# daxiongpro/EPNet

Hardware: AMD Instinct MI355X
Metric: SA-stack points/sec per GPU (16384-pt KITTI scene) + % HBM roofline (higher is better)
Workload: dtype f32

## Files before the change

### epnet_amd/csrc/group.hip

```cpp

#include <type_traits>

#include "common.h"
#include "spatial.h"
#include "runsum.h"

namespace epnet {

constexpr int kGThreads = 256;
constexpr int kGChan = 16;

__global__ __launch_bounds__(kGThreads) void gather_rows_vec4_kernel(int c, int n, int p, size_t ostride,
                                                                     const float *__restrict__ points,
                                                                     const int *__restrict__ idx,
                                                                     float *__restrict__ out) {
    int wg_x, wg_y, bs;
    xcd_scene_map3(wg_x, wg_y, bs);
    const int c0 = wg_y * kGChan;
    const int q4 = wg_x * kGThreads + threadIdx.x;
    if (q4 * 4 >= p) return;
    const int4 id = *reinterpret_cast<const int4 *>(idx + (size_t)bs * p + (size_t)q4 * 4);
    const int cend = min(c, c0 + kGChan);
    const float *src = points + ((size_t)bs * c + c0) * n;
    float *dst = out + (size_t)bs * ostride + (size_t)c0 * p + (size_t)q4 * 4;
// ... 224 lines not shown
#pragma unroll 1
        for (int set = 0; set < 2; ++set) {
            const int p = set ? p1 : p0;
            const int *ix = (set ? idx1 : idx0) + (size_t)bs * p;
            float *dst_base = (set ? out1 : out0) + (size_t)bs * (set ? ostride1 : ostride0) + (size_t)c0 * p;
            if (p > 0) serve_span<QUAD, decltype(g)::value, decltype(u)::value>(s_rows, nr, n, ix, 0, p, dst_base, p);
        }
    });
}

__global__ __launch_bounds__(kGThreads) void scatter_rows_lds_kernel(int c, int n, int p, int rows, size_t gstride,
                                                                     const float *__restrict__ grad_out,
                                                                     const int *__restrict__ idx,
                                                                     float *__restrict__ grad_points) {
    extern __shared__ float acc[];
    const int bs = blockIdx.y;
    const int c0 = blockIdx.x * rows;
    const int nr = min(rows, c - c0);
    for (int e = threadIdx.x; e < nr * n; e += kGThreads) acc[e] = 0.f;
    __syncthreads();
    const int *ix = idx + (size_t)bs * p;
    const float *go = grad_out + (size_t)bs * gstride + (size_t)c0 * p;
    for (int q = threadIdx.x; q < p; q += kGThreads) {
        const int id = ix[q];
        for (int r = 0; r < nr; ++r) atomicAdd(&acc[r * n + id], go[(size_t)r * p + q]);
    }
    __syncthreads();
    float *gp = grad_points + ((size_t)bs * c + c0) * n;
    for (int e = threadIdx.x; e < nr * n; e += kGThreads) gp[e] += acc[e];
}

__global__ __launch_bounds__(kGThreads) void scatter_rows_atomic_kernel(int c, int n, int p, size_t gstride,
                                                                        const float *__restrict__ grad_out,
                                                                        const int *__restrict__ idx,
                                                                        float *__restrict__ grad_points) {
    const int bs = blockIdx.z, ci = blockIdx.y;
    const int q = blockIdx.x * kGThreads + threadIdx.x;
    if (q >= p) return;
    atomicAdd(grad_points + ((size_t)bs * c + ci) * n + idx[(size_t)bs * p + q],
              grad_out[(size_t)bs * gstride + (size_t)ci * p + q]);
}

__global__ __launch_bounds__(kGThreads) void group_xyz_centred_kernel(int n, int npoints, int nsample, size_t ostride,
                                                                      const float *__restrict__ xyz,
                                                                      const float *__restrict__ new_xyz,
                                                                      const int *__restrict__ idx, float *__restrict__ out) {
    int wg_x, bs;
    xcd_scene_map(wg_x, bs);
    const int p = npoints * nsample;
    const int q = wg_x * kGThreads + threadIdx.x;
    if (q >= p) return;
    const int id = idx[(size_t)bs * p + q];
    const int ci = q / nsample;
    const float *pt = xyz + ((size_t)bs * n + id) * 3;
    const float *ce = new_xyz + ((size_t)bs * npoints + ci) * 3;
    float *dst = out + (size_t)bs * ostride + q;
    dst[0] = pt[0] - ce[0];
    dst[(size_t)p] = pt[1] - ce[1];
    dst[(size_t)p * 2] = pt[2] - ce[2];
}

__global__ __launch_bounds__(kGThreads) void group_xyz_centred_vec4_kernel(int n, int npoints, int nsample, size_t ostride,
                                                                           const float *__restrict__ xyz,
                                                                           const float *__restrict__ new_xyz,
                                                                           const int *__restrict__ idx,
                                                                           float *__restrict__ out) {
    int wg_x, bs;
    xcd_scene_map(wg_x, bs);
    const int p = npoints * nsample;
    const int q = (wg_x * kGThreads + threadIdx.x) * 4;
    if (q >= p) return;
    const int4 id = *reinterpret_cast<const int4 *>(idx + (size_t)bs * p + q);
    const float *base = xyz + (size_t)bs * n * 3;
    const float *ce = new_xyz + ((size_t)bs * npoints + q / nsample) * 3;
    const float cx = ce[0], cy = ce[1], cz = ce[2];
    const float *p0 = base + (size_t)id.x * 3, *p1 = base + (size_t)id.y * 3, *p2 = base + (size_t)id.z * 3,
                *p3 = base + (size_t)id.w * 3;
    float *dst = out + (size_t)bs * ostride + q;
    *reinterpret_cast<float4 *>(dst) = make_float4(p0[0] - cx, p1[0] - cx, p2[0] - cx, p3[0] - cx);
    *reinterpret_cast<float4 *>(dst + (size_t)p) = make_float4(p0[1] - cy, p1[1] - cy, p2[1] - cy, p3[1] - cy);
    *reinterpret_cast<float4 *>(dst + (size_t)p * 2) = make_float4(p0[2] - cz, p1[2] - cz, p2[2] - cz, p3[2] - cz);
}

__global__ __launch_bounds__(kGLdsThreads) void group_linear_lds_kernel(int c, int n, int npoints, int nsample, int rows, int tile,
                                                                        const float *__restrict__ z, const float *__restrict__ xyz,
                                                                        const float *__restrict__ new_xyz, const int *__restrict__ idx,
                                                                        const float *__restrict__ wx, const float *__restrict__ bias,
                                                                        float *__restrict__ out) {
    extern __shared__ float s_rows[];
    const int bs = blockIdx.z;
    const int c0 = blockIdx.y * rows;
    const int nr = min(rows, c - c0);
    const int p = npoints * nsample;
    const float *src = z + ((size_t)bs * c + c0) * n;
    const int total = nr * n;
    if ((n & 3) == 0 && ((uintptr_t)src & 15) == 0) {
        const float4 *src4 = reinterpret_cast<const float4 *>(src);
        float4 *dst4 = reinterpret_cast<float4 *>(s_rows);
        EPNET_STAGE_PRAGMA
        for (int e = threadIdx.x; e < total / 4; e += kGLdsThreads) dst4[e] = src4[e];
    } else {
        for (int e = threadIdx.x; e < total; e += kGLdsThreads) s_rows[e] = src[e];
    }
    __syncthreads();
    const int q_begin = blockIdx.x * tile, q_end = min(p, q_begin + tile);
    const int *ix = idx + (size_t)bs * p;
    const float *pts = xyz + (size_t)bs * n * 3;
    float *dst_base = out + ((size_t)bs * c + c0) * p;
    for (int q = q_begin + threadIdx.x * 4; q < q_end; q += kGLdsThreads * 4) {
        const int4 id = *reinterpret_cast<const int4 *>(ix + q);
        const float *ce = new_xyz + ((size_t)bs * npoints + q / nsample) * 3;
        const float cx = ce[0], cy = ce[1], cz = ce[2];
        const float *p0 = pts + (size_t)id.x * 3, *p1 = pts + (size_t)id.y * 3, *p2 = pts + (size_t)id.z * 3, *p3 = pts + (size_t)id.w * 3;
        const float dx0 = p0[0] - cx, dy0 = p0[1] - cy, dz0 = p0[2] - cz;
        const float dx1 = p1[0] - cx, dy1 = p1[1] - cy, dz1 = p1[2] - cz;
        const float dx2 = p2[0] - cx, dy2 = p2[1] - cy, dz2 = p2[2] - cz;
        const float dx3 = p3[0] - cx, dy3 = p3[1] - cy, dz3 = p3[2] - cz;
        float *dst = dst_base + q;
        const float *row = s_rows;
#pragma unroll 2
        for (int r = 0; r < nr; ++r) {
            const float w0 = wx[(c0 + r) * 3], w1 = wx[(c0 + r) * 3 + 1], w2 = wx[(c0 + r) * 3 + 2];
            float4 v;
            v.x = row[id.x] + (w0 * dx0 + w1 * dy0 + w2 * dz0);
            v.y = row[id.y] + (w0 * dx1 + w1 * dy1 + w2 * dz1);
            v.z = row[id.z] + (w0 * dx2 + w1 * dy2 + w2 * dz2);
            v.w = row[id.w] + (w0 * dx3 + w1 * dy3 + w2 * dz3);
            if (bias) {
                const float bv = bias[c0 + r];
                v.x += bv; v.y += bv; v.z += bv; v.w += bv;
            }
            store_stream(dst, v.x, v.y, v.z, v.w);
            row += n;
            dst += p;
        }
    }
}

__global__ __launch_bounds__(kGThreads) void group_linear_scalar_kernel(int c, int n, int npoints, int nsample,
                                                                        const float *__restrict__ z, const float *__restrict__ xyz,
                                                                        const float *__restrict__ new_xyz, const int *__restrict__ idx,
                                                                        const float *__restrict__ wx, const float *__restrict__ bias,
                                                                        float *__restrict__ out) {
    const int bs = blockIdx.z;
    const int c0 = blockIdx.y * kGChan;
    const int p = npoints * nsample;
    const int q = blockIdx.x * kGThreads + threadIdx.x;
    if (q >= p) return;
    const int id = idx[(size_t)bs * p + q];
    const float *pt = xyz + ((size_t)bs * n + id) * 3;
    const float *ce = new_xyz + ((size_t)bs * npoints + q / nsample) * 3;
    const float dx = pt[0] - ce[0], dy = pt[1] - ce[1], dz = pt[2] - ce[2];
    const int cend = min(c, c0 + kGChan);
    for (int ci = c0; ci < cend; ++ci) {
        float v = z[((size_t)bs * c + ci) * n + id] + (wx[ci * 3] * dx + wx[ci * 3 + 1] * dy + wx[ci * 3 + 2] * dz);
        if (bias) v += bias[ci];
        out[((size_t)bs * c + ci) * p + q] = v;
    }
}

constexpr int kGwRows = 8;
__global__ __launch_bounds__(kGThreads) void group_linear_grad_w_kernel(int c, int n, int npoints, int nsample, int tile,
                                                                        const float *__restrict__ grad_out,
                                                                        const float *__restrict__ xyz,
                                                                        const float *__restrict__ new_xyz,
                                                                        const int *__restrict__ idx, float *__restrict__ grad_w) {
// ... 258 lines not shown
}

static int launch_group_xyz(int b, int n, int npoints, int nsample, long long p, size_t ostride, const float *xyz,
                            const float *new_xyz, const int *idx, float *out, hipStream_t s) {
    if (nsample % 4 == 0 && (((uintptr_t)idx | (uintptr_t)out) % 16 == 0) && (ostride % 4 == 0))
        hipLaunchKernelGGL(group_xyz_centred_vec4_kernel, dim3((unsigned)div_up64(p / 4, kGThreads), b), dim3(kGThreads), 0, s, n,
                           npoints, nsample, ostride, xyz, new_xyz, idx, out);
    else
        hipLaunchKernelGGL(group_xyz_centred_kernel, dim3((unsigned)div_up64(p, kGThreads), b), dim3(kGThreads), 0, s, n, npoints,
                           nsample, ostride, xyz, new_xyz, idx, out);
    return check_launch("group_concat xyz");
}

extern "C" int epnet_group_concat(int b, int c, int n, int npoints, int nsample, const float *xyz, const float *new_xyz,
                                  const float *features, const int *idx, float *out, int use_xyz, epnet_stream_t stream) {
    EPNET_REQUIRE(b >= 0 && c >= 0 && n >= 0 && npoints >= 0 && nsample >= 0);
    EPNET_REQUIRE(use_xyz || c > 0);
    const long long p = (long long)npoints * nsample;
    if (b == 0 || p == 0) return EPNET_OK;
    EPNET_REQUIRE(idx && out && (c == 0 || features) && (!use_xyz || (xyz && new_xyz)));
    EPNET_REQUIRE(n > 0);
    if (p > 0x7fffffffll || b > 65535) return EPNET_ELIMIT;
    hipStream_t s = (hipStream_t)stream;
    const int ch0 = use_xyz ? 3 : 0;
    const size_t ostride = (size_t)(ch0 + c) * (size_t)p;
    if (use_xyz) {
        int rc = launch_group_xyz(b, n, npoints, nsample, p, ostride, xyz, new_xyz, idx, out, s);
        if (rc) return rc;
    }
    if (c == 0) return EPNET_OK;
    return launch_gather_rows(b, c, n, p, features, idx, out + (size_t)ch0 * p, s, "group_concat features", ostride);
}

extern "C" size_t epnet_group_concat_workspace_bytes(int b, int c, int n, int npoints, int nsample) {
    return gather_pm_ws_bytes(b, c, n, (long long)npoints * nsample);
}

extern "C" int epnet_group_concat_ws(int b, int c, int n, int npoints, int nsample, const float *xyz, const float *new_xyz,
                                     const float *features, const int *idx, float *out, int use_xyz, void *workspace,
                                     size_t workspace_bytes, epnet_stream_t stream) {
    const long long p = (long long)npoints * nsample;
    const size_t need = gather_pm_ws_bytes(b, c, n, p);
    if (need == 0 || !workspace || ((uintptr_t)workspace & 15))
        return epnet_group_concat(b, c, n, npoints, nsample, xyz, new_xyz, features, idx, out, use_xyz, stream);
    if (workspace_bytes < need) return EPNET_ENOMEM;
    EPNET_REQUIRE(b >= 0 && n > 0 && npoints >= 0 && nsample >= 0 && features && idx && out && (!use_xyz || (xyz && new_xyz)));
    if (p > 0x7fffffffll || b > 65535) return EPNET_ELIMIT;
    const int ch0 = use_xyz ? 3 : 0;
    const size_t ostride = (size_t)(ch0 + c) * (size_t)p;
    if (use_xyz) {
        int rc = launch_group_xyz(b, n, npoints, nsample, p, ostride, xyz, new_xyz, idx, out, (hipStream_t)stream);
        if (rc) return rc;
    }
    return launch_gather_rows_pm(b, c, n, p, features, idx, out + (size_t)ch0 * p, ostride, workspace, (hipStream_t)stream,
                                 "group_concat features");
}

extern "C" int epnet_group_concat_multi(int b, int c, int n, int npoints, int nscales, const int *nsamples, const float *xyz,
                                        const float *new_xyz, const float *features, const int *const *idx, float *const *out,
                                        int use_xyz, epnet_stream_t stream) {
    EPNET_REQUIRE(nscales >= 0 && (nscales == 0 || (nsamples && idx && out)));
    hipStream_t s = (hipStream_t)stream;
    const int ch0 = use_xyz ? 3 : 0;
    constexpr int kLdsBudget = EPNET_GATHER_LDS_BUDGET_KB * 1024;
    bool fused = nscales == 2 && c >= 8 && b > 0 && n > 0 && npoints > 0 && (size_t)n * 4 <= (size_t)kLdsBudget && features && b <= 65535;
    int rows = 0;
    bool quad = false;
    if (fused) {
        rows = kLdsBudget / (n * 4);
        if (rows > c) rows = c;
        if (rows > 32) rows = 32;
        quad = (c & 3) == 0 && (n & 3) == 0 && rows >= 4 && ((uintptr_t)features & 15) == 0;
        if (quad) rows &= ~3;
        long long p_both = 0;
        for (int k = 0; k < 2 && fused; ++k) {
            const long long p = (long long)npoints * nsamples[k];
            fused = p > 0 && p <= 0x7fffffffll && p % 4 == 0 && idx[k] && out[k] &&
                    (((uintptr_t)idx[k] | (uintptr_t)out[k]) % 16 == 0) && ((size_t)(ch0 + c) * (size_t)p) % 4 == 0;
            p_both += p;
        }
        fused = fused && p_both >= kGatherLds2MinPositions;
        fused = fused && (long long)b * div_up(c, rows) >= 512;
    }
    if (!fused) {
        for (int k = 0; k < nscales; ++k) {
            const int rc = epnet_group_concat(b, c, n, npoints, nsamples[k], xyz, new_xyz, features, idx[k], out[k], use_xyz, stream);
            if (rc) return rc;
        }
        return EPNET_OK;
    }
    size_t ostride[2];
    int pk[2];
    for (int k = 0; k < 2; ++k) {
        pk[k] = npoints * nsamples[k];
        ostride[k] = (size_t)(ch0 + c) * (size_t)pk[k];
        if (!use_xyz) continue;
        EPNET_REQUIRE(xyz && new_xyz);
        const long long p = pk[k];
        if (nsamples[k] % 4 == 0)
            hipLaunchKernelGGL(group_xyz_centred_vec4_kernel, dim3((unsigned)div_up64(p / 4, kGThreads), b), dim3(kGThreads), 0, s,
                               n, npoints, nsamples[k], ostride[k], xyz, new_xyz, idx[k], out[k]);
        else
            hipLaunchKernelGGL(group_xyz_centred_kernel, dim3((unsigned)div_up64(p, kGThreads), b), dim3(kGThreads), 0, s, n,
                               npoints, nsamples[k], ostride[k], xyz, new_xyz, idx[k], out[k]);
        const int rc = check_launch("group_concat_multi xyz");
        if (rc) return rc;
    }
    if (quad)
        hipLaunchKernelGGL(gather_rows_lds2_kernel<true>, dim3(div_up(c, rows), b), dim3(kGLdsThreads), (size_t)rows * n * 4, s, c, n,
                           rows, features, pk[0], ostride[0], idx[0], out[0] + (size_t)ch0 * pk[0], pk[1], ostride[1], idx[1],
                           out[1] + (size_t)ch0 * pk[1]);
    else
        hipLaunchKernelGGL(gather_rows_lds2_kernel<false>, dim3(div_up(c, rows), b), dim3(kGLdsThreads), (size_t)rows * n * 4, s, c, n,
                           rows, features, pk[0], ostride[0], idx[0], out[0] + (size_t)ch0 * pk[0], pk[1], ostride[1], idx[1],
                           out[1] + (size_t)ch0 * pk[1]);
    return check_launch("group_concat_multi");
}

extern "C" int epnet_group_concat_grad(int b, int c, int n, int npoints, int nsample, const float *grad_out, const int *idx,
                                       float *grad_features, int use_xyz, epnet_stream_t stream) {
    EPNET_REQUIRE(b >= 0 && c >= 0 && n >= 0 && npoints >= 0 && nsample >= 0);
    const long long p = (long long)npoints * nsample;
    if (b == 0 || c == 0 || p == 0) return EPNET_OK;
    const int ch0 = use_xyz ? 3 : 0;
    const size_t gstride = (size_t)(ch0 + c) * (size_t)p;
    return launch_scatter_rows(b, c, n, p, grad_out + (size_t)ch0 * p, idx, grad_features, (hipStream_t)stream,
                               "group_concat_grad", gstride);
}

extern "C" size_t epnet_group_points_grad_workspace_bytes(int b, int n, int npoints, int nsample) {
    return scatter_ws_bytes(b, n, (long long)npoints * nsample);
}

extern "C" int epnet_group_points_grad_ws(int b, int c, int n, int npoints, int nsample, const float *grad_out,
                                          const int *idx, float *grad_points, void *workspace, size_t workspace_bytes,
                                          epnet_stream_t stream) {
    EPNET_REQUIRE(b >= 0 && c >= 0 && n >= 0 && npoints >= 0 && nsample >= 0);
    const long long p = (long long)npoints * nsample;
    if (scatter_ws_bytes(b, n, p) == 0 || ((uintptr_t)grad_out & 15))
        return launch_scatter_rows(b, c, n, p, grad_out, idx, grad_points, (hipStream_t)stream, "group_points_grad");
    return launch_scatter_rows_csr(b, c, n, p, grad_out, idx, grad_points, workspace, workspace_bytes, (hipStream_t)stream,
                                   "group_points_grad", 0);
}

extern "C" int epnet_group_concat_grad_ws(int b, int c, int n, int npoints, int nsample, const float *grad_out,
                                          const int *idx, float *grad_features, int use_xyz, void *workspace,
                                          size_t workspace_bytes, epnet_stream_t stream) {
    EPNET_REQUIRE(b >= 0 && c >= 0 && n >= 0 && npoints >= 0 && nsample >= 0);
    const long long p = (long long)npoints * nsample;
    if (b == 0 || c == 0 || p == 0) return EPNET_OK;
    const int ch0 = use_xyz ? 3 : 0;
    const size_t gstride = (size_t)(ch0 + c) * (size_t)p;
    if (scatter_ws_bytes(b, n, p) == 0 || ((uintptr_t)grad_out & 15))
        return launch_scatter_rows(b, c, n, p, grad_out + (size_t)ch0 * p, idx, grad_features, (hipStream_t)stream,
                                   "group_concat_grad", gstride);
    return launch_scatter_rows_csr(b, c, n, p, grad_out + (size_t)ch0 * p, idx, grad_features, workspace, workspace_bytes,
                                   (hipStream_t)stream, "group_concat_grad", gstride);
}

extern "C" int epnet_group_linear(int b, int c, int n, int npoints, int nsample, const float *xyz, const float *new_xyz,
                                  const float *z, const int *idx, const float *w_xyz, const float *bias, float *out,
                                  epnet_stream_t stream) {
    EPNET_REQUIRE(b >= 0 && c >= 0 && n >= 0 && npoints >= 0 && nsample >= 0);
    const long long p = (long long)npoints * nsample;
    if (b == 0 || c == 0 || p == 0) return EPNET_OK;
    EPNET_REQUIRE(xyz && new_xyz && z && idx && w_xyz && out && n > 0);
    if (p > 0x7fffffffll || b > 65535 || div_up(c, kGChan) > 65535) return EPNET_ELIMIT;
    hipStream_t s = (hipStream_t)stream;
    constexpr int kLdsBudget = EPNET_GATHER_LDS_BUDGET_KB * 1024;
    const bool vec = nsample % 4 == 0 && (((uintptr_t)idx | (uintptr_t)out) % 16 == 0);
    if (vec && c >= 8 && (size_t)n * 4 <= (size_t)kLdsBudget && p >= 1024) {
        int rows = kLdsBudget / (n * 4);
        if (rows > c) rows = c;
        if (rows > 32) rows = 32;
        const int chunks = div_up(c, rows);
        int tiles = div_up(1024, b * chunks);
        const int max_tiles = (int)(p / 1024);
        if (tiles > max_tiles) tiles = max_tiles;
        if (tiles < 1) tiles = 1;
// ... 34 lines not shown
```

### epnet_amd/sa_stack.py

```python
import os

import torch

from . import pointnet2_cuda as ext

RPN_NPOINTS = (4096, 1024, 256, 64)
RPN_RADII = ((0.1, 0.5), (0.5, 1.0), (1.0, 2.0), (2.0, 4.0))
RPN_NSAMPLES = ((16, 32), (16, 32), (16, 32), (16, 32))
RPN_FEAT_CHANNELS = (0, 96, 256, 512)
RPN_FP = ((1024, 64, 256), (512, 256, 1024), (512, 1024, 4096), (256, 4096, 16384))


CONFIGS = {
    2: dict(n=16384, npoints=RPN_NPOINTS, radii=RPN_RADII, nsamples=RPN_NSAMPLES, feat_channels=RPN_FEAT_CHANNELS),
    5: dict(n=65536, npoints=(16384,), radii=((0.5,),), nsamples=((64,),), feat_channels=(64,)),
}


def sa_algorithmic_bytes(n=16384, npoints=RPN_NPOINTS, nsamples=RPN_NSAMPLES, feat_channels=RPN_FEAT_CHANNELS):
    out = {"fps": 0, "gather": 0, "ball_query": 0, "group_xyz": 0, "group_feat": 0}
    cur = n
    for lvl, m in enumerate(npoints):
        out["fps"] += cur * 12 + m * 4
        out["gather"] += m * 4 + 3 * cur * 4 + 3 * m * 4
        for ns in nsamples[lvl]:
            out["ball_query"] += cur * 12 + m * 12 + m * ns * 4
            out["group_xyz"] += m * ns * 4 + 3 * cur * 4 + 3 * m * ns * 4
            c = feat_channels[lvl]
            if c:
                out["group_feat"] += m * ns * 4 + c * cur * 4 + c * m * ns * 4
        cur = m
    out["total"] = sum(out.values())
    return out


def fp_algorithmic_bytes(fp=RPN_FP):
    out = {"three_nn": 0, "three_interpolate": 0}
    for c, m, n in fp:
        out["three_nn"] += n * 12 + m * 12 + n * 24
        out["three_interpolate"] += c * m * 4 + n * 24 + c * n * 4
    out["total"] = sum(out.values())
    return out


class SAStack:
    def __init__(self, batch, n=16384, device="cuda", npoints=RPN_NPOINTS, radii=RPN_RADII, nsamples=RPN_NSAMPLES,
                 feat_channels=RPN_FEAT_CHANNELS, with_fp=False, fp=RPN_FP, seed=0, overlap=True, fused=True,
                 shared_index=True, pipelined=False, fused_sampling=False, queries_in_s=None, s_query_levels=None, stages=None):
        self.batch, self.n = batch, n
        if stages is None:
            stages = int(os.environ.get("EPNET_SA_STAGES", "2"))
        self.stages = 3 if (pipelined and stages == 3 and fused_sampling and fused and shared_index) else (2 if pipelined else 1)
        self.ring = self.stages
        self.overlap = overlap
        self.fused = fused
        self.shared_index = shared_index
        self.pipelined = pipelined
        self.fused_sampling = fused_sampling
        env_q = int(os.environ.get("EPNET_SA_QUERIES_IN_S", "1"))
        env_lv = os.environ.get("EPNET_SA_S_QUERY_LEVELS")
        every = frozenset(range(len(npoints)))
        if not pipelined:
            chosen = frozenset()
        elif s_query_levels is not None:
            chosen = frozenset(int(v) for v in s_query_levels)
        elif queries_in_s is not None:
            chosen = every if queries_in_s else frozenset()
        elif env_lv is not None:
            chosen = frozenset(int(v) for v in env_lv.split(",") if v.strip())
        elif self.stages == 3:
            chosen = every
        elif env_q == 2 or (env_q == 1 and with_fp):
            chosen = every
        elif env_q == 1 and batch * n >= 240 * 16384:
            chosen = every - {0, 1}
        else:
            chosen = frozenset()
        self.s_query_levels = chosen & every
        self.queries_in_s = self.s_query_levels == every
        self.chain = bool(int(os.environ.get("EPNET_SA_CHAIN", "1"))) and fused_sampling
        self.fuse_gather = int(os.environ.get("EPNET_SA_FUSE_GATHER", "1"))
        self._deferred = None
        self._next_built = None
        self.s_first = bool(int(os.environ.get("EPNET_SA_S_FIRST", "0" if self.s_query_levels else "1")))
        self.tail_scales = int(os.environ.get("EPNET_SA_TAIL_SCALES", "0"))
        self.multi_query = bool(int(os.environ.get("EPNET_SA_MULTI_QUERY", "1")))
        self.multi_group = bool(int(os.environ.get("EPNET_SA_MULTI_GROUP", "1")))
        self.ordered_query = bool(int(os.environ.get("EPNET_SA_ORDERED_QUERY", "1")))
        self.side = None
        self.npoints, self.radii, self.nsamples, self.feat_channels = npoints, radii, nsamples, feat_channels
        self.with_fp, self.fp = with_fp, fp
        dev = torch.device(device)
        g = torch.Generator().manual_seed(seed)
        f32, i32 = torch.float32, torch.int32
        self.levels = []
        cur = n
        for lvl, m in enumerate(npoints):
            c = feat_channels[lvl]
            index_bytes = ext.scene_index_bytes(batch, cur) if shared_index else 0
            L = {
                "n": cur, "m": m, "c": c,
                "xyz_t_sets": [torch.empty((batch, 3, cur), dtype=f32, device=dev) for _ in range(self.ring if not fused else 1)],
                "temp": torch.empty((batch, cur), dtype=f32, device=dev),
                "fps_idx_sets": ([torch.empty((batch, m), dtype=i32, device=dev) for _ in range(3)] if self.stages == 3 else None),
                "fps_idx": None,
                "new_xyz_t": torch.empty((batch, 3, m), dtype=f32, device=dev),
                "sets": [{"new_xyz": torch.empty((batch, m, 3), dtype=f32, device=dev),
                          "index": (torch.empty((index_bytes,), dtype=torch.uint8, device=dev) if index_bytes else None),
                          "prefix": torch.zeros((batch,), dtype=i32, device=dev),
                          "centre_index": (torch.empty((ext.scene_index_bytes(batch, m),), dtype=torch.uint8, device=dev)
                                           if (shared_index and lvl + 1 == len(npoints) and ext.scene_index_bytes(batch, m)) else None)}
                         for _ in range(self.ring)],
                "features": (torch.randn((batch, c, cur), generator=g, dtype=f32).to(dev) if c else None),
                "scales": [],
            }
            for radius, ns in zip(radii[lvl], nsamples[lvl]):
                S = {"radius": radius, "ns": ns, "idx": torch.empty((batch, m, ns), dtype=i32, device=dev)}
                S["idx_sets"] = [S["idx"]] + ([torch.empty((batch, m, ns), dtype=i32, device=dev) for _ in range(self.ring - 1)]
                                              if lvl in self.s_query_levels else [])
                if fused:
                    S["grouped"] = torch.empty((batch, 3 + c, m, ns), dtype=f32, device=dev)
                    ws_bytes = ext.group_concat_workspace_bytes(batch, c, cur, m, ns)
                    S["workspace"] = torch.empty((ws_bytes,), dtype=torch.uint8, device=dev) if ws_bytes else None
                else:
                    S["grouped_xyz"] = torch.empty((batch, 3, m, ns), dtype=f32, device=dev)
                    S["grouped_feat"] = torch.empty((batch, c, m, ns), dtype=f32, device=dev) if c else None
                L["scales"].append(S)
            if L["fps_idx_sets"] is None:
                one = torch.empty((batch, m), dtype=i32, device=dev)
                L["fps_idx_sets"] = [one] * self.ring
            L["fps_idx"] = L["fps_idx_sets"][0]
            self.levels.append(L)
            cur = m
        self.fp_bufs = []
        if with_fp:
            for c, m, nn_ in fp:
                sets = [{"dist2": torch.empty((batch, nn_, 3), dtype=f32, device=dev),
                         "idx": torch.empty((batch, nn_, 3), dtype=i32, device=dev),
                         "weight": torch.empty((batch, nn_, 3), dtype=f32, device=dev)} for _ in range(self.ring)]
                self.fp_bufs.append({
                    "c": c, "m": m, "n": nn_,
                    "known_feats": torch.randn((batch, c, m), generator=g, dtype=f32).to(dev),
                    "sets": sets,
                    "dist2": sets[0]["dist2"], "idx": sets[0]["idx"],
                    "out": torch.empty((batch, c, nn_), dtype=f32, device=dev),
                })
        self.graphs = []
        self.replays = 0
        self.inputs = []
        self._prev_xyz = None

    @property
    def static_xyz(self):
        if self.pipelined and self.inputs:
            raise AttributeError("a pipelined stack has one input buffer per parity: use stack.inputs / stack.input_buffer()")
        return self.inputs[0] if self.inputs else None

    def input_buffer(self, step=None):
        step = self.replays if step is None else step
        return self.inputs[step % len(self.inputs)]

    def owners(self):
        if self.stages == 3:
            raise RuntimeError("three stages: see owners3()")
        p = (self.replays - 1) & 1 if self.pipelined else 0
        return p, (1 - p if self.pipelined else 0)

# ... 75 lines not shown
                                     self._idx(S, parity), S["grouped"], True, S.get("workspace"))
        else:
            ext.group_points_wrapper(b, 3, n, m, S["ns"], L["xyz_t_sets"][parity], self._idx(S, parity), S["grouped_xyz"])
            if L["c"]:
                ext.group_points_wrapper(b, L["c"], n, m, S["ns"], L["features"], self._idx(S, parity), S["grouped_feat"])

    def _query_level(self, L, cur_xyz, parity):
        P = L["sets"][parity]
        centre_index = (self._centre_index(L, parity)
                        if (self.ordered_query and L["n"] > 16384 and P["index"] is not None and len(L["scales"]) <= 2) else None)
        if centre_index is not None:
            ext.ball_query_ordered_wrapper(self.batch, L["n"], L["m"], [S["radius"] for S in L["scales"]],
                                         [S["ns"] for S in L["scales"]], P["new_xyz"], cur_xyz, P["index"], centre_index,
                                         [self._idx(S, parity) for S in L["scales"]])
        elif P["index"] is not None and self.multi_query:
            ext.ball_query_multi_wrapper(self.batch, L["n"], L["m"], [S["radius"] for S in L["scales"]],
                                         [S["ns"] for S in L["scales"]], P["new_xyz"], cur_xyz, P["index"],
                                         [self._idx(S, parity) for S in L["scales"]])
        else:
            for S in L["scales"]:
                self._query_scale(L, S, cur_xyz, parity)

    def _centre_index(self, L, parity):
        lvl = self.levels.index(L)
        if lvl + 1 < len(self.levels):
            return self.levels[lvl + 1]["sets"][parity]["index"] if self.shared_index else None
        own = L["sets"][parity].get("centre_index")
        if own is not None:
            ext.scene_index_build_wrapper(self.batch, L["m"], L["sets"][parity]["new_xyz"], own)
        return own

    def _group_scales(self, L, cur_xyz, parity):
        if self.fused and self.multi_group and len(L["scales"]) > 1:
            ext.group_concat_multi_wrapper(self.batch, L["c"], L["n"], L["m"], [S["ns"] for S in L["scales"]], cur_xyz,
                                           L["sets"][parity]["new_xyz"], L["features"], [self._idx(S, parity) for S in L["scales"]],
                                           [S["grouped"] for S in L["scales"]], True)
        else:
            for S in L["scales"]:
                self._group_scale(L, S, cur_xyz, parity)

    def _group_level(self, L, cur_xyz, parity):
        self._query_level(L, cur_xyz, parity)
        self._group_scales(L, cur_xyz, parity)

    def _side_stream(self, device):
        if self.side is None:
            self.side = torch.cuda.Stream(device=device)
        return self.side

    def run(self, xyz):
        main = torch.cuda.current_stream(xyz.device)
        side = self._side_stream(xyz.device) if self.overlap else None
        cur_xyz = xyz
        built = False
        for lvl, L in enumerate(self.levels):
            new_xyz = self._sample_level(L, cur_xyz, 0, index_built=built)
            built = False
            nxt = self.levels[lvl + 1] if lvl + 1 < len(self.levels) else None
            if self.ordered_query and L["n"] > 16384 and nxt is not None and nxt["sets"][0]["index"] is not None:
                ext.scene_index_build_wrapper(self.batch, L["m"], new_xyz, nxt["sets"][0]["index"])
                built = True
            if side is not None:
                side.wait_stream(main)
                with torch.cuda.stream(side):
                    self._group_level(L, cur_xyz, 0)
            else:
                self._group_level(L, cur_xyz, 0)
            cur_xyz = new_xyz
        if side is not None:
            main.wait_stream(side)
        if self.with_fp:
            self._run_fp(xyz, 0)

    def run_pipelined(self, xyz, prev_xyz, step):
        parity = step & 1
        main = torch.cuda.current_stream(xyz.device)
        side = self._side_stream(xyz.device)
        first = self.levels[0]
        if first["sets"][parity]["index"] is not None:
            ext.scene_index_build_wrapper(self.batch, first["n"], xyz, first["sets"][parity]["index"])
        forked = torch.cuda.Event()
        forked.record(main)
        s_cur = xyz
        if self.s_first:
            s_cur = self._sample_level(first, xyz, parity, index_built=True, defer_ok=True)
        side.wait_event(forked)
        with torch.cuda.stream(side):
            inputs = [prev_xyz] + [L["sets"][1 - parity]["new_xyz"] for L in self.levels[:-1]]
            in_s = self.s_query_levels
            deep = list(enumerate(zip(self.levels, inputs)))[1:]
            for lvl, (L, cur) in deep[:1]:
                if lvl not in in_s:
                    self._query_level(L, cur, 1 - parity)
                self._group_scales(L, cur, 1 - parity)
            for lvl, (L, cur) in deep[1:]:
                if lvl not in in_s:
                    self._query_level(L, cur, 1 - parity)
            for lvl, (L, cur) in deep[1:]:
                self._group_scales(L, cur, 1 - parity)
            if 0 in in_s:
                self._group_scales(first, prev_xyz, 1 - parity)
            elif self.tail_scales == 0:
                self._group_level(first, prev_xyz, 1 - parity)
            else:
                for S in first["scales"][self.tail_scales:]:
                    self._query_scale(first, S, prev_xyz, 1 - parity)
                    self._group_scale(first, S, prev_xyz, 1 - parity)
            if self.with_fp:
                self._interpolate_fp(1 - parity)
        for L in self.levels[(1 if self.s_first else 0):]:
            s_cur = self._sample_level(L, s_cur, parity, index_built=L is first, defer_ok=True)
        if self.with_fp:
            self._search_fp(xyz, parity)
        if self.s_query_levels:
            self._queries_of(xyz, parity)
        for S in first["scales"][:(0 if 0 in self.s_query_levels else self.tail_scales)]:
            self._query_scale(first, S, prev_xyz, 1 - parity)
            self._group_scale(first, S, prev_xyz, 1 - parity)
        main.wait_stream(side)

    def run_pipelined3(self, clouds, step):
        p, q, r = step % 3, (step - 1) % 3, (step - 2) % 3
        main = torch.cuda.current_stream(clouds[p].device)
        side = self._side_stream(clouds[p].device)
        third = self._third_stream(clouds[p].device)
        first = self.levels[0]
        ext.scene_index_build_wrapper(self.batch, first["n"], clouds[p], first["sets"][p]["index"])
        forked = torch.cuda.Event()
        forked.record(main)
        self._deferred = self._next_built = None
        self._sample_level(first, clouds[p], p, index_built=True, defer_ok=True)
        s1_deferred = self._deferred is not None
        s1_built = self._next_built is not None
        self._deferred = self._next_built = None
        side.wait_event(forked)
        with torch.cuda.stream(side):
            inputs = [clouds[r]] + [L["sets"][r]["new_xyz"] for L in self.levels[:-1]]
            order = list(zip(self.levels, inputs))
            for lvl, (L, cur) in enumerate(order[1:], start=1):
                if lvl not in self.s_query_levels:
                    self._query_level(L, cur, r)
                self._group_scales(L, cur, r)
            if 0 not in self.s_query_levels:
                self._query_level(first, clouds[r], r)
            self._group_scales(first, clouds[r], r)
            if self.with_fp:
                self._interpolate_fp(r)
        third.wait_event(forked)
        with torch.cuda.stream(third):
            self._deferred = (clouds[q], 0, q) if s1_deferred else None
            self._next_built = (1, q) if s1_built else None
            cur = first["sets"][q]["new_xyz"]
            for L in self.levels[1:]:
                cur = self._sample_level(L, cur, q, defer_ok=True)
            self._deferred = self._next_built = None
            if self.with_fp:
                self._search_fp(clouds[q], q)
            self._queries_of(clouds[q], q)
        main.wait_stream(side)
        main.wait_stream(third)

    def _third_stream(self, device):
        if getattr(self, "third", None) is None:
            self.third = torch.cuda.Stream(device=device)
        return self.third

    def _queries_of(self, xyz, parity):
        cur = xyz
        for lvl, L in enumerate(self.levels):
            if lvl in self.s_query_levels:
                self._query_level(L, cur, parity)
            cur = L["sets"][parity]["new_xyz"]

    def _search_fp(self, xyz, parity):
        b = self.batch
        xyzs = [xyz] + [L["sets"][parity]["new_xyz"] for L in self.levels]
        indices = [L["sets"][parity]["index"] for L in self.levels] + [None]
        for k, F in enumerate(self.fp_bufs):
            P = F["sets"][parity if len(F["sets"]) > 1 else 0]
            known = xyzs[len(self.levels) - k]
            unknown = xyzs[len(self.levels) - k - 1]
            k_index, u_index = indices[len(self.levels) - k], indices[len(self.levels) - k - 1]
            if k_index is not None:
                ext.three_nn_indexed_wrapper(b, F["n"], F["m"], unknown, known, u_index, k_index, P["dist2"], P["idx"])
            else:
                ext.three_nn_wrapper(b, F["n"], F["m"], unknown, known, P["dist2"], P["idx"])
            inv = 1.0 / (torch.sqrt(P["dist2"]) + 1e-8)
            torch.div(inv, torch.sum(inv, dim=2, keepdim=True), out=P["weight"])
            F["dist2"], F["idx"] = P["dist2"], P["idx"]

    def _interpolate_fp(self, parity):
        b = self.batch
        for F in self.fp_bufs:
            P = F["sets"][parity if len(F["sets"]) > 1 else 0]
            ext.three_interpolate_wrapper(b, F["c"], F["m"], F["n"], F["known_feats"], P["idx"], P["weight"], F["out"])

    def _run_fp(self, xyz, parity):
        self._search_fp(xyz, parity)
        self._interpolate_fp(parity)

    def _prime(self, clouds):
        for parity in range(self.ring):
            xyz = cur = clouds[parity]
            self._deferred = self._next_built = None
            for L in self.levels:
                cur = self._sample_level(L, cur, parity, defer_ok=True)
            self._deferred = self._next_built = None
            if self.with_fp:
                self._search_fp(xyz, parity)
            if self.s_query_levels:
                self._queries_of(xyz, parity)

    def _step_eager(self, k):
        if self.stages == 3:
            self.run_pipelined3(self.inputs, k)
        elif self.pipelined:
            self.run_pipelined(self.inputs[k & 1], self.inputs[1 - (k & 1)], k)
        else:
            self.run(self.inputs[0])

    def capture(self, xyz, xyz_other=None, xyz_third=None):
        self.inputs = [xyz.clone()]
        if self.pipelined:
            self.inputs.append((xyz if xyz_other is None else xyz_other).clone())
        if self.stages == 3:
            self.inputs.append((xyz if xyz_third is None else xyz_third).clone())
        s = torch.cuda.Stream()
        s.wait_stream(torch.cuda.current_stream())
        period = 1
        with torch.cuda.stream(s):
            if self.pipelined:
                self._prime(self.inputs)
        if self.pipelined:
            period = self.ring
        with torch.cuda.stream(s):
            for k in range(max(2, period)):
                self._step_eager(k)
        torch.cuda.current_stream().wait_stream(s)
        torch.cuda.synchronize()
        self.graphs = []
        for k in range(period):
            g = torch.cuda.CUDAGraph()
            with torch.cuda.graph(g):
                self._step_eager(k)
            self.graphs.append(g)
        self.replays = 0
        return self.graphs[0]

    def replay(self, xyz=None):
        if xyz is not None:
            self.input_buffer().copy_(xyz)
        self.graphs[self.replays % len(self.graphs)].replay()
        self.replays += 1
# ... 22 lines not shown
```

### profiles/micro/step_tails.py

```python
import csv, statistics, sys
rows = list(csv.DictReader(open(sys.argv[1])))
skip = int(sys.argv[2]) if len(sys.argv) > 2 else 3
rows.sort(key=lambda r: int(r["Start_Timestamp"]))
name = lambda r: r["Kernel_Name"].replace("epnet::", "").replace("void ", "").split("(")[0]
anchors = [i for i, r in enumerate(rows) if "fps_indexed_kernel<8, 32" in r["Kernel_Name"]]
steps = []
for a, b in zip(anchors[skip:-skip - 1], anchors[skip + 1:-skip]):
    t0, t1 = int(rows[a]["Start_Timestamp"]), int(rows[b]["Start_Timestamp"])
    fps_end = int(rows[a]["End_Timestamp"])
    s_queue = rows[a]["Queue_Id"]
    inside = [r for r in rows[a:b] if int(r["Start_Timestamp"]) < t1]
    s_end = max(int(r["End_Timestamp"]) for r in inside if r["Queue_Id"] == s_queue)
    g = [r for r in inside if r["Queue_Id"] != s_queue and "bq_index_kernel<1024" not in r["Kernel_Name"]]
    g_end = max(int(r["End_Timestamp"]) for r in g if int(r["Start_Timestamp"]) > fps_end - 500000)
    q1 = [r for r in g if "bq_query2_kernel<8" in r["Kernel_Name"]]
    d = {"step": t1 - t0, "fps L1": fps_end - t0, "S tail (fps end -> S end)": s_end - fps_end, "S end": s_end - t0, "G end": g_end - t0}
    if q1:
        d["L1 query start - fps end"] = int(q1[0]["Start_Timestamp"]) - fps_end
    for r in inside:
        if int(r["Start_Timestamp"]) >= fps_end - 300000 and "gather_rows" not in r["Kernel_Name"]:
            k = ("S " if r["Queue_Id"] == s_queue else "G ") + name(r)
            d[k] = d.get(k, 0) + int(r["End_Timestamp"]) - int(r["Start_Timestamp"])
    steps.append(d)
print("%d steady steps" % len(steps))
for k in steps[0]:
    v = [s[k] / 1e6 for s in steps if k in s]
    print("%-58s median %7.3f  min %7.3f  max %7.3f ms" % (k[:58], statistics.median(v), min(v), max(v)))
```

Before: 1.484 billion.

## Merge two-scale xyz grouping into one launch and add L1 query placement modes

Adds a single kernel that writes centred xyz for both sample scales in one launch. It loads each point as a 12-byte struct instead of three scalar loads and replaces two per-scale launches on both the fused and unfused grouping paths. It also adds an EPNET_SA_L1_QUERY option (free/gated/branch) that can move the level-1 ball query onto a third stream, or gate level-1 grouping behind level-1 sampling, to reshape cross-stream overlap. The default placement is "free", so the scheduling change is off unless enabled. The profiling scripts are extended to attribute kernels by stage.

```diff
diff --git a/epnet_amd/csrc/group.hip b/epnet_amd/csrc/group.hip
--- a/epnet_amd/csrc/group.hip
+++ b/epnet_amd/csrc/group.hip
@@ -330,6 +330,37 @@
     *reinterpret_cast<float4 *>(dst + (size_t)p * 2) = make_float4(p0[2] - cz, p1[2] - cz, p2[2] - cz, p3[2] - cz);
 }
 
+struct xyz_row {
+    float x, y, z;
+};
+struct xyz_scale {
+    int nsample, p;
+    size_t ostride;
+    const int *idx;
+    float *out;
+};
+__global__ __launch_bounds__(kGThreads) void group_xyz_centred_multi_kernel(int n, int npoints, int wgs0, xyz_scale s0, xyz_scale s1,
+                                                                            const float *__restrict__ xyz,
+                                                                            const float *__restrict__ new_xyz) {
+    int wg_x, bs;
+    xcd_scene_map(wg_x, bs);
+    const bool second = wg_x >= wgs0;
+    const int nsample = second ? s1.nsample : s0.nsample, p = second ? s1.p : s0.p;
+    const size_t ostride = second ? s1.ostride : s0.ostride;
+    const int *__restrict__ idx = second ? s1.idx : s0.idx;
+    float *__restrict__ out = second ? s1.out : s0.out;
+    const int q = ((second ? wg_x - wgs0 : wg_x) * kGThreads + threadIdx.x) * 4;
+    if (q >= p) return;
+    const int4 id = *reinterpret_cast<const int4 *>(idx + (size_t)bs * p + q);
+    const xyz_row *rows = reinterpret_cast<const xyz_row *>(xyz) + (size_t)bs * n;
+    const xyz_row ce = reinterpret_cast<const xyz_row *>(new_xyz)[(size_t)bs * npoints + q / nsample];
+    const xyz_row r0 = rows[id.x], r1 = rows[id.y], r2 = rows[id.z], r3 = rows[id.w];
+    float *dst = out + (size_t)bs * ostride + q;
+    *reinterpret_cast<float4 *>(dst) = make_float4(r0.x - ce.x, r1.x - ce.x, r2.x - ce.x, r3.x - ce.x);
+    *reinterpret_cast<float4 *>(dst + (size_t)p) = make_float4(r0.y - ce.y, r1.y - ce.y, r2.y - ce.y, r3.y - ce.y);
+    *reinterpret_cast<float4 *>(dst + (size_t)p * 2) = make_float4(r0.z - ce.z, r1.z - ce.z, r2.z - ce.z, r3.z - ce.z);
+}
+
 __global__ __launch_bounds__(kGLdsThreads) void group_linear_lds_kernel(int c, int n, int npoints, int nsample, int rows, int tile,
                                                                         const float *__restrict__ z, const float *__restrict__ xyz,
                                                                         const float *__restrict__ new_xyz, const int *__restrict__ idx,
@@ -754,9 +785,36 @@
         fused = fused && p_both >= kGatherLds2MinPositions;
         fused = fused && (long long)b * div_up(c, rows) >= 512;
     }
+    bool paired = use_xyz && nscales == 2 && b > 0 && b <= 65535 && c >= 0 && n > 0 && npoints > 0 && xyz && new_xyz &&
+                  (c == 0 || features);
+    long long wgs[2] = {0, 0};
+    for (int k = 0; k < 2 && paired; ++k) {
+        const long long p = (long long)npoints * nsamples[k];
+        paired = nsamples[k] > 0 && nsamples[k] % 4 == 0 && p <= 0x7fffffffll && idx[k] && out[k] &&
+                 (((uintptr_t)idx[k] | (uintptr_t)out[k]) % 16 == 0) && ((size_t)(ch0 + c) * (size_t)p) % 4 == 0;
+        wgs[k] = div_up64(p / 4, kGThreads);
+    }
+    paired = paired && (wgs[0] + wgs[1]) * b <= 0x7fffffffll;
+    if (paired) {
+        xyz_scale sc[2];
+        for (int k = 0; k < 2; ++k) {
+            const int p = npoints * nsamples[k];
+            sc[k] = xyz_scale{nsamples[k], p, (size_t)(ch0 + c) * (size_t)p, idx[k], out[k]};
+        }
+        hipLaunchKernelGGL(group_xyz_centred_multi_kernel, dim3((unsigned)(wgs[0] + wgs[1]), b), dim3(kGThreads), 0, s, n, npoints,
+                           (int)wgs[0], sc[0], sc[1], xyz, new_xyz);
+        const int rc = check_launch("group_concat_multi xyz");
+        if (rc) return rc;
+    }
     if (!fused) {
         for (int k = 0; k < nscales; ++k) {
-            const int rc = epnet_group_concat(b, c, n, npoints, nsamples[k], xyz, new_xyz, features, idx[k], out[k], use_xyz, stream);
+            int rc = EPNET_OK;
+            if (!paired)
+                rc = epnet_group_concat(b, c, n, npoints, nsamples[k], xyz, new_xyz, features, idx[k], out[k], use_xyz, stream);
+            else if (c > 0)
+                rc = launch_gather_rows(b, c, n, (long long)npoints * nsamples[k], features, idx[k],
+                                        out[k] + (size_t)ch0 * npoints * nsamples[k], s, "group_concat features",
+                                        (size_t)(ch0 + c) * (size_t)npoints * nsamples[k]);
             if (rc) return rc;
         }
         return EPNET_OK;
@@ -766,7 +824,7 @@
     for (int k = 0; k < 2; ++k) {
         pk[k] = npoints * nsamples[k];
         ostride[k] = (size_t)(ch0 + c) * (size_t)pk[k];
-        if (!use_xyz) continue;
+        if (!use_xyz || paired) continue;
         EPNET_REQUIRE(xyz && new_xyz);
         const long long p = pk[k];
         if (nsamples[k] % 4 == 0)
diff --git a/epnet_amd/sa_stack.py b/epnet_amd/sa_stack.py
--- a/epnet_amd/sa_stack.py
+++ b/epnet_amd/sa_stack.py
@@ -46,7 +46,8 @@
 class SAStack:
     def __init__(self, batch, n=16384, device="cuda", npoints=RPN_NPOINTS, radii=RPN_RADII, nsamples=RPN_NSAMPLES,
                  feat_channels=RPN_FEAT_CHANNELS, with_fp=False, fp=RPN_FP, seed=0, overlap=True, fused=True,
-                 shared_index=True, pipelined=False, fused_sampling=False, queries_in_s=None, s_query_levels=None, stages=None):
+                 shared_index=True, pipelined=False, fused_sampling=False, queries_in_s=None, s_query_levels=None, stages=None,
+                 l1_query=None):
         self.batch, self.n = batch, n
         if stages is None:
             stages = int(os.environ.get("EPNET_SA_STAGES", "2"))
@@ -76,13 +77,22 @@
             chosen = every - {0, 1}
         else:
             chosen = frozenset()
-        self.s_query_levels = chosen & every
+        chosen = chosen & every
+        placement = l1_query if l1_query is not None else os.environ.get("EPNET_SA_L1_QUERY", "free")
+        if placement not in ("free", "gated", "branch"):
+            raise ValueError("EPNET_SA_L1_QUERY / l1_query: free, gated or branch, not %r" % (placement,))
+        if self.stages != 2 or 0 in chosen or int(os.environ.get("EPNET_SA_TAIL_SCALES", "0")):
+            placement = "free"
+        if placement == "branch" and n > 16384:
+            placement = "free"
+        self.l1_query = placement
+        self.s_query_levels = (chosen | {0}) if placement == "branch" else chosen
         self.queries_in_s = self.s_query_levels == every
         self.chain = bool(int(os.environ.get("EPNET_SA_CHAIN", "1"))) and fused_sampling
         self.fuse_gather = int(os.environ.get("EPNET_SA_FUSE_GATHER", "1"))
         self._deferred = None
         self._next_built = None
-        self.s_first = bool(int(os.environ.get("EPNET_SA_S_FIRST", "0" if self.s_query_levels else "1")))
+        self.s_first = bool(int(os.environ.get("EPNET_SA_S_FIRST", "0" if chosen else "1")))
         self.tail_scales = int(os.environ.get("EPNET_SA_TAIL_SCALES", "0"))
         self.multi_query = bool(int(os.environ.get("EPNET_SA_MULTI_QUERY", "1")))
         self.multi_group = bool(int(os.environ.get("EPNET_SA_MULTI_GROUP", "1")))
@@ -324,8 +334,11 @@
         forked = torch.cuda.Event()
         forked.record(main)
         s_cur = xyz
+        sampled = 0
+        placement = self.l1_query
         if self.s_first:
             s_cur = self._sample_level(first, xyz, parity, index_built=True, defer_ok=True)
+            sampled = 1
         side.wait_event(forked)
         with torch.cuda.stream(side):
             inputs = [prev_xyz] + [L["sets"][1 - parity]["new_xyz"] for L in self.levels[:-1]]
@@ -342,6 +355,8 @@
                 self._group_scales(L, cur, 1 - parity)
             if 0 in in_s:
                 self._group_scales(first, prev_xyz, 1 - parity)
+            elif placement == "gated":
+                pass
             elif self.tail_scales == 0:
                 self._group_level(first, prev_xyz, 1 - parity)
             else:
@@ -350,16 +365,34 @@
                     self._group_scale(first, S, prev_xyz, 1 - parity)
             if self.with_fp:
                 self._interpolate_fp(1 - parity)
-        for L in self.levels[(1 if self.s_first else 0):]:
+        third = None
+        if placement != "free":
+            while sampled < 1 or (placement == "branch" and self._deferred is not None):
+                s_cur = self._sample_level(self.levels[sampled], s_cur, parity, index_built=sampled == 0, defer_ok=True)
+                sampled += 1
+            l1_sampled = torch.cuda.Event()
+            l1_sampled.record(main)
+            if placement == "gated":
+                side.wait_event(l1_sampled)
+                with torch.cuda.stream(side):
+                    self._group_level(first, prev_xyz, 1 - parity)
+            else:
+                third = self._third_stream(xyz.device)
+                third.wait_event(l1_sampled)
+                with torch.cuda.stream(third):
+                    self._query_level(first, xyz, parity)
+        for L in self.levels[sampled:]:
             s_cur = self._sample_level(L, s_cur, parity, index_built=L is first, defer_ok=True)
         if self.with_fp:
             self._search_fp(xyz, parity)
         if self.s_query_levels:
-            self._queries_of(xyz, parity)
+            self._queries_of(xyz, parity, skip=(0,) if placement == "branch" else ())
         for S in first["scales"][:(0 if 0 in self.s_query_levels else self.tail_scales)]:
             self._query_scale(first, S, prev_xyz, 1 - parity)
             self._group_scale(first, S, prev_xyz, 1 - parity)
         main.wait_stream(side)
+        if third is not None:
+            main.wait_stream(third)
 
     def run_pipelined3(self, clouds, step):
         p, q, r = step % 3, (step - 1) % 3, (step - 2) % 3
@@ -407,10 +440,10 @@
             self.third = torch.cuda.Stream(device=device)
         return self.third
 
-    def _queries_of(self, xyz, parity):
+    def _queries_of(self, xyz, parity, skip=()):
         cur = xyz
         for lvl, L in enumerate(self.levels):
-            if lvl in self.s_query_levels:
+            if lvl in self.s_query_levels and lvl not in skip:
                 self._query_level(L, cur, parity)
             cur = L["sets"][parity]["new_xyz"]
 
diff --git a/profiles/micro/group_xyz_pmc.py b/profiles/micro/group_xyz_pmc.py
--- /dev/null
+++ b/profiles/micro/group_xyz_pmc.py
@@ -0,0 +1,16 @@
+import sys, os
+sys.path.insert(0, os.path.dirname(os.path.dirname(os.path.dirname(os.path.abspath(__file__)))) if len(sys.argv) < 2 else sys.argv[1])
+import torch
+from epnet_amd import pointnet2_cuda as ext, synth
+
+b, n, m, nss = 256, 16384, 4096, (16, 32)
+dev = "cuda:0"
+xyz = synth.scenes("kitti", b, n, seed=1).to(dev)
+g = torch.Generator().manual_seed(3)
+centres = xyz[:, :m].contiguous()
+idxs = [torch.randint(0, n, (b, m, ns), generator=g, dtype=torch.int32).to(dev) for ns in nss]
+outs = [torch.empty((b, 3, m, ns), device=dev) for ns in nss]
+for _ in range(3):
+    ext.group_concat_multi_wrapper(b, 0, n, m, list(nss), xyz, centres, None, idxs, outs, True)
+torch.cuda.synchronize()
+print("done")
diff --git a/profiles/micro/step_tails.py b/profiles/micro/step_tails.py
--- a/profiles/micro/step_tails.py
+++ b/profiles/micro/step_tails.py
@@ -3,26 +3,70 @@
 skip = int(sys.argv[2]) if len(sys.argv) > 2 else 3
 rows.sort(key=lambda r: int(r["Start_Timestamp"]))
 name = lambda r: r["Kernel_Name"].replace("epnet::", "").replace("void ", "").split("(")[0]
+
+
+def stage(r):
+    n = r["Kernel_Name"]
+    if "bq_query2_kernel<8" in n:
+        return "Q1"
+    if "bq_index_kernel<1024" in n:
+        return "-"
+    return "G" if ("gather_rows" in n or "group_xyz" in n or "bq_query2_kernel<2" in n) else "S"
+
+
 anchors = [i for i, r in enumerate(rows) if "fps_indexed_kernel<8, 32" in r["Kernel_Name"]]
 steps = []
 for a, b in zip(anchors[skip:-skip - 1], anchors[skip + 1:-skip]):
     t0, t1 = int(rows[a]["Start_Timestamp"]), int(rows[b]["Start_Timestamp"])
     fps_end = int(rows[a]["End_Timestamp"])
-    s_queue = rows[a]["Queue_Id"]
     inside = [r for r in rows[a:b] if int(r["Start_Timestamp"]) < t1]
-    s_end = max(int(r["End_Timestamp"]) for r in inside if r["Queue_Id"] == s_queue)
-    g = [r for r in inside if r["Queue_Id"] != s_queue and "bq_index_kernel<1024" not in r["Kernel_Name"]]
-    g_end = max(int(r["End_Timestamp"]) for r in g if int(r["Start_Timestamp"]) > fps_end - 500000)
-    q1 = [r for r in g if "bq_query2_kernel<8" in r["Kernel_Name"]]
+    s_end = max(int(r["End_Timestamp"]) for r in inside if stage(r) == "S")
+    g_end = max(int(r["End_Timestamp"]) for r in inside if stage(r) == "G" and "bq_query2_kernel<2" not in r["Kernel_Name"])
+    q1 = [r for r in inside if stage(r) == "Q1"]
     d = {"step": t1 - t0, "fps L1": fps_end - t0, "S tail (fps end -> S end)": s_end - fps_end, "S end": s_end - t0, "G end": g_end - t0}
     if q1:
-        d["L1 query start - fps end"] = int(q1[0]["Start_Timestamp"]) - fps_end
+        q_start, q_end = int(q1[0]["Start_Timestamp"]), int(q1[0]["End_Timestamp"])
+        d["L1 query start - fps end"] = q_start - fps_end
+        d["L1 query"] = q_end - q_start
+        d["L1 query end"] = q_end - t0
+        d["L1 query under the fps"] = max(0, min(q_end, fps_end) - q_start)
     for r in inside:
-        if int(r["Start_Timestamp"]) >= fps_end - 300000 and "gather_rows" not in r["Kernel_Name"]:
-            k = ("S " if r["Queue_Id"] == s_queue else "G ") + name(r)
+        if int(r["Start_Timestamp"]) >= fps_end - 300000 and "gather_rows" not in r["Kernel_Name"] and stage(r) in "SG":
+            k = stage(r) + " " + name(r)
             d[k] = d.get(k, 0) + int(r["End_Timestamp"]) - int(r["Start_Timestamp"])
+    d["_rows"] = (t0, rows[max(a - 2, 0):b])
     steps.append(d)
 print("%d steady steps" % len(steps))
 for k in steps[0]:
+    if k == "_rows":
+        continue
     v = [s[k] / 1e6 for s in steps if k in s]
     print("%-58s median %7.3f  min %7.3f  max %7.3f ms" % (k[:58], statistics.median(v), min(v), max(v)))
+
+
+def pearson(x, y):
+    if len(x) < 3 or len(set(x)) < 2 or len(set(y)) < 2:
+        return float("nan")
+    mx, my = statistics.fmean(x), statistics.fmean(y)
+    sxy = sum((a - mx) * (b - my) for a, b in zip(x, y))
+    return sxy / (sum((a - mx) ** 2 for a in x) * sum((b - my) ** 2 for b in y)) ** 0.5
+
+
+per = [s for s in steps if "L1 query" in s]
+if per:
+    print("\nstep by step [ms]: fps L1, L1 query start - fps end, L1 query, L1 query under the fps, step")
+    for s in per:
+        print("  %7.3f  %+7.3f  %7.3f  %7.3f  %7.3f" % tuple(s[k] / 1e6 for k in ("fps L1", "L1 query start - fps end", "L1 query",
+                                                                                   "L1 query under the fps", "step")))
+    settled = [s for s in per if s["step"] <= 1.03 * statistics.median(t["step"] for t in per)]
+    for what, sel in (("all", per), ("settled", settled)):
+        over = [s["L1 query under the fps"] / 1e6 for s in sel]
+        print("correlation with the overlap (L1 query under the fps), %s %d steps: fps L1 %+.2f, step %+.2f, L1 query %+.2f" % (
+            what, len(sel), pearson([s["fps L1"] / 1e6 for s in sel], over), pearson([s["step"] / 1e6 for s in sel], over),
+            pearson([s["L1 query"] / 1e6 for s in sel], over)))
+mid = sorted(steps, key=lambda s: s["step"])[len(steps) // 2]
+t0, tl = mid["_rows"]
+print("\nthe steady step of median length (%.3f ms): stage, kernel, queue, start, end, duration [ms from the level-1 FPS start]" % (mid["step"] / 1e6))
+for r in tl:
+    st, en = int(r["Start_Timestamp"]), int(r["End_Timestamp"])
+    print("  %-2s %-46s q%-2s %8.3f %8.3f %7.3f" % (stage(r), name(r)[:46], r["Queue_Id"], (st - t0) / 1e6, (en - t0) / 1e6, (en - st) / 1e6))
```

Result: no change. 1.484 billion (-0.0%).
